# toandaominh1997/EfficientDet.Pytorch

Measured on AMD Instinct MI355X. Metric: images/sec EfficientDet-D0 512px fwd+bwd, higher is better.
Workload: dtype f32_hf16x3_bwd_bf16x3

## Files before the change

efficientdet/pytorch_amd/_lib.py:

```python
import ctypes as C
import os

import torch

HERE = os.path.dirname(os.path.abspath(__file__))
LIB_PATH = os.environ.get('EFFDET_HIP_LIB') or os.path.join(os.path.dirname(os.path.abspath(__file__)), 'libeffdet_hip.so')
MAX_SEG = 5
MAX_CONV_SEG = 10
ABI_VERSION = 11
F32, BF16, F32_BF16X3, F32_SPLIT = 0, 1, 2, 3
F32_HSPLIT = 4
ACT_NONE, ACT_RELU, ACT_SWISH, ACT_SIGMOID = 0, 1, 2, 3
RES_NONE, RES_ADD, RES_RELU_MASK, RES_SWISH_GRAD = 0, 1, 2, 3
TUNE_IGEMM_BIG, TUNE_IGEMM_BIG_MIN_M, TUNE_SPLIT_PERS, TUNE_IGEMM_KORD, TUNE_SPLIT_KORD = 0, 1, 2, 3, 4

_ERR = {-1: 'EFFDET_EINVAL', -2: 'EFFDET_ELAUNCH', -3: 'EFFDET_EUNSUPPORTED'}


class Seg(C.Structure):
    _fields_ = [('H', C.c_int), ('W', C.c_int), ('Ho', C.c_int), ('Wo', C.c_int),
                ('in_off', C.c_longlong), ('in_bstride', C.c_longlong),
                ('out_off', C.c_longlong), ('out_bstride', C.c_longlong)]


class ConvDesc(C.Structure):
    _fields_ = [('x', C.c_void_p), ('w', C.c_void_p), ('y', C.c_void_p), ('z', C.c_void_p), ('res', C.c_void_p),
                ('scale', C.c_void_p), ('shift', C.c_void_p), ('rowscale', C.c_void_p),
                ('bc_scale', C.c_void_p), ('bc_shift', C.c_void_p),
                ('dtype', C.c_int), ('out_f32', C.c_int),
                ('B', C.c_int), ('Cin', C.c_int), ('Cout', C.c_int), ('KH', C.c_int), ('KW', C.c_int),
                ('stride', C.c_int), ('pad_t', C.c_int), ('pad_l', C.c_int),
                ('ldx', C.c_int), ('ldy', C.c_int), ('act', C.c_int), ('res_mode', C.c_int),
                ('nseg', C.c_int), ('seg', Seg * MAX_CONV_SEG), ('w_image_stride', C.c_longlong), ('y_split', C.c_void_p), ('range_flag', C.c_void_p),
                ('seg_w', C.c_void_p * MAX_CONV_SEG), ('seg_shift', C.c_void_p * MAX_CONV_SEG)]


class WgradDesc(C.Structure):
    _fields_ = [('x', C.c_void_p), ('dz', C.c_void_p), ('dw', C.c_void_p), ('dbias', C.c_void_p),
                ('dtype', C.c_int),
                ('B', C.c_int), ('Cin', C.c_int), ('Cout', C.c_int), ('KH', C.c_int), ('KW', C.c_int),
                ('stride', C.c_int), ('pad_t', C.c_int), ('pad_l', C.c_int),
                ('ldx', C.c_int), ('lddz', C.c_int), ('nseg', C.c_int), ('image_splits', C.c_int), ('seg', Seg * MAX_SEG)]


class PrepJob(C.Structure):
    _fields_ = [('a', C.c_void_p), ('b', C.c_void_p), ('c', C.c_void_p), ('d', C.c_void_p), ('out', C.c_void_p),
                ('kind', C.c_int), ('dtype', C.c_int), ('n0', C.c_int), ('n1', C.c_int), ('n2', C.c_int), ('n3', C.c_int),
                ('n4', C.c_int), ('eps', C.c_float)]


class UnpackJob(C.Structure):
    _fields_ = [(n, C.c_void_p) for n in ('g', 'scale', 'w_oihw', 'dw_oihw', 'wsum', 'dsum_part', 'mean', 'invstd', 'dgamma', 'dbeta',
                                          'dbias_out', 'slab_scale', 'slab_cscale')] + \
               [(n, C.c_int) for n in ('accumulate', 'Cout', 'Cin', 'KH', 'KW', 'Cin_pad', 'nslabs', 'slabs_per_scale')]


class SeParamJob(C.Structure):
    _fields_ = [(n, C.c_void_p) for n in ('du', 'dmid', 'sw', 'pool', 'dw1', 'db1', 'dw2', 'db2')] + \
               [('B', C.c_int), ('C', C.c_int), ('Cse', C.c_int), ('inv_hw', C.c_float)]


class DwUnpackJob(C.Structure):
    _fields_ = [(n, C.c_void_p) for n in ('g_kkc', 'scale', 'w_c1kk', 'dw_c1kk', 'wsum', 'dsum', 'mean', 'invstd', 'dgamma', 'dbeta')] + \
               [('C', C.c_int), ('kk', C.c_int)]


class _TailUnion(C.Union):
# ... 296 lines not shown
```

efficientdet/pytorch_amd/csrc/conv_igemm.hip:

```cpp
#include "common.h"
#include "../../../include/effdet_live_tiles.h"
#include "../../../include/effdet_needed_tiles.h"
#include "../../../include/effdet_conv_plan.h"
#include "../../../include/effdet_gate_operand.h"
#include <stdlib.h>

#ifndef EFFDET_IGEMM_BIG_DEFAULT
#define EFFDET_IGEMM_BIG_DEFAULT 1
#endif

namespace {

struct SegD {
  int H, W, Ho, Wo, M, tile_start;
  long long in_off, in_bs, out_off, out_bs;
  unsigned x_bytes;
  long long w_off;
  long long sh_off;
};

struct ConvK {
  const void* x; const void* w; void* y; void* z; const void* res;
  const float* scale; const float* shift; const float* rowscale;
  const float* bc_scale; const float* bc_shift;
  int Cin, Cout, KW, stride, pad_t, pad_l;
  int ldx, ldy;
  int Kc;
  int cpt;
  int act, res_mode, out_f32, vec_ok;
  int out_split;
  int* range_flag;
  void* ysplit;
  int nseg, mtiles, ntiles;
  unsigned w_bytes;
  int kord;
  long long w_img_bytes;
  const unsigned char* live;
  int live_tile0;
  const unsigned char* needed;
  int needed_tile0;
  const float* a_gate;
  SegD seg[EFFDET_MAX_CONV_SEG];
};

constexpr int BM = 128;
typedef float f32x16 __attribute__((ext_vector_type(16)));

template <typename T> struct Mma;
template <> struct Mma<bf16_t> {
  static __device__ __forceinline__ void run(const uint4& a, const uint4& b, f32x4& c) {
    c = __builtin_amdgcn_mfma_f32_16x16x32_bf16(__builtin_bit_cast(bf16x8, a), __builtin_bit_cast(bf16x8, b), c, 0, 0, 0);
  }
};
struct MmaH {
  static __device__ __forceinline__ void run(const uint4& a, const uint4& b, f32x4& c) {
    c = __builtin_amdgcn_mfma_f32_16x16x32_f16(__builtin_bit_cast(f16x8, a), __builtin_bit_cast(f16x8, b), c, 0, 0, 0);
  }
};
template <> struct Mma<float> {
  static __device__ __forceinline__ void run(const uint4& a, const uint4& b, f32x4& c) {
    c = __builtin_amdgcn_mfma_f32_16x16x4f32(__uint_as_float(a.x), __uint_as_float(b.x), c, 0, 0, 0);
    c = __builtin_amdgcn_mfma_f32_16x16x4f32(__uint_as_float(a.y), __uint_as_float(b.y), c, 0, 0, 0);
    c = __builtin_amdgcn_mfma_f32_16x16x4f32(__uint_as_float(a.z), __uint_as_float(b.z), c, 0, 0, 0);
    c = __builtin_amdgcn_mfma_f32_16x16x4f32(__uint_as_float(a.w), __uint_as_float(b.w), c, 0, 0, 0);
  }
};

template <typename T, int BN, int WAVES_N, int NWAVES, int SPLIT = 0, int NS = 2, int M32 = 0, int GATE = 0>
__global__ __launch_bounds__(NWAVES * 64, (SPLIT == 3 && NWAVES == 4) ? 3 : 1) void conv_igemm_kernel(const ConvK p) {
  static_assert(!SPLIT || sizeof(T) == 4, "bf16x3 splitting applies to fp32 storage");
  static_assert(!M32 || SPLIT == 2, "the 32x32x16 form is built for the split layout");
  static_assert(SPLIT != 3 || NS == 2, "f16x3: two stages");
  static_assert(NS == 2 || !M32, "deep staging is not built for the 32x32 tile loop");
  static_assert(!GATE || (SPLIT == 0 && sizeof(T) == 4), "the operand gate is built for the exact-fp32 form");
  constexpr int CE = Elem<T>::CE;
  constexpr int NTHREADS = NWAVES * 64;
  constexpr int WAVES_M = NWAVES / WAVES_N;
  constexpr int WTM = BM / WAVES_M, WTN = BN / WAVES_N;
  constexpr int MT = WTM / 16, NT = WTN / 16;
  constexpr int XLD = BM * 8;
  constexpr int WLD = BN * 8;
  constexpr int RSTEP = NTHREADS / 8;
  constexpr int XROWS = BM / RSTEP;
  constexpr int WROWS = (BN + RSTEP - 1) / RSTEP;

  extern __shared__ __attribute__((aligned(16))) uint4 smem[];
  uint4* xs = smem;
  uint4* ws = smem + NS * XLD;

  const int tid = threadIdx.x;
  const int lane = tid & 63, wave = tid >> 6;
  const int wm0 = (wave / WAVES_N) * WTM, wn0 = (wave % WAVES_N) * WTN;

  int tile = xcd_remap(blockIdx.x, gridDim.x);
  if constexpr (SPLIT == 2) {
    if (p.live) {
      const int b = blockIdx.x, whole = (p.mtiles >> 3) << 3;
      if (b < whole * p.ntiles) {
        const int i = b >> 3, j = i / p.ntiles;
        tile = (j * 8 + (b & 7)) * p.ntiles + (i - j * p.ntiles);
      } else tile = b;
    }
  }
  if constexpr (SPLIT == 3) {
    if (p.needed) {
      const int b = blockIdx.x, whole = (p.mtiles >> 3) << 3;
      if (b < whole * p.ntiles) {
        const int i = b >> 3, j = i / p.ntiles;
        tile = (j * 8 + (b & 7)) * p.ntiles + (i - j * p.ntiles);
      } else tile = b;
    }
  }
  const int mt = tile / p.ntiles, nt = tile - mt * p.ntiles;
  int si = 0;
#pragma unroll
  for (int s = 1; s < EFFDET_MAX_CONV_SEG; ++s)
    if (s < p.nseg && mt >= p.seg[s].tile_start) si = s;
  const SegD sg = p.seg[si];
  const int m_base = (mt - sg.tile_start) * BM;
  const int n_base = nt * BN;
  const int HoWo = sg.Ho * sg.Wo;

  if constexpr (SPLIT == 2) {
    if (p.live && mt >= p.live_tile0 && p.live[mt - p.live_tile0] == 0) {
      if (p.res_mode == EFFDET_RES_ADD) return;
      const int rows = min(BM, sg.M - m_base), nch = min(BN, p.Cout - n_base);
      if (p.vec_ok) {
        const int q4 = nch >> 2;
        for (int i = tid; i < rows * q4; i += NTHREADS) {
          const int row = i / q4, c = i - row * q4;
          const int m = m_base + row, bi = m / HoWo, pix = m - bi * HoWo;
          *(uint4*)((float*)p.y + sg.out_off + (long long)bi * sg.out_bs + (long long)pix * p.ldy + n_base + 4 * c) = make_uint4(0u, 0u, 0u, 0u);
        }
      } else {
        for (int i = tid; i < rows * nch; i += NTHREADS) {
          const int row = i / nch, c = i - row * nch;
          const int m = m_base + row, bi = m / HoWo, pix = m - bi * HoWo;
          ((float*)p.y)[sg.out_off + (long long)bi * sg.out_bs + (long long)pix * p.ldy + n_base + c] = 0.f;
        }
      }
      return;
    }
  }

  if constexpr (SPLIT == 3) {
    if (p.needed && mt >= p.needed_tile0 && p.needed[mt - p.needed_tile0] == 0) {
      const int rows = min(BM, sg.M - m_base), nch = min(BN, p.Cout - n_base);
      if (p.vec_ok) {
        const int q4 = nch >> 2;
        for (int i = tid; i < rows * q4; i += NTHREADS) {
          const int row = i / q4, c = i - row * q4;
          const int m = m_base + row, bi = m / HoWo, pix = m - bi * HoWo;
          const long long o = sg.out_off + (long long)bi * sg.out_bs + (long long)pix * p.ldy + n_base + 4 * c;
          *(uint4*)((float*)p.y + o) = make_uint4(0u, 0u, 0u, 0u);
          if (p.ysplit) *(uint4*)((float*)p.ysplit + o) = make_uint4(0u, 0u, 0u, 0u);
        }
      } else {
        for (int i = tid; i < rows * nch; i += NTHREADS) {
          const int row = i / nch, c = i - row * nch;
          const int m = m_base + row, bi = m / HoWo, pix = m - bi * HoWo;
          ((float*)p.y)[sg.out_off + (long long)bi * sg.out_bs + (long long)pix * p.ldy + n_base + c] = 0.f;
        }
      }
      return;
    }
  }

  constexpr unsigned ES = sizeof(T);
  const long long w_img = p.w_img_bytes ? (long long)(m_base / HoWo) * p.w_img_bytes : 0ll;
  const u32x4_t rx = make_srd_raw((const T*)p.x + sg.in_off, sg.x_bytes), rw = make_srd_raw((const char*)p.w + w_img + sg.w_off, p.w_bytes);
  const unsigned xs_a = lds_addr(xs), ws_a = lds_addr(ws);
  const int kc = (tid & 7) ^ ((tid >> 4) & 7), r0 = tid >> 3;
  const int wrow0 = __builtin_amdgcn_readfirstlane(wave) * 8;
  unsigned xoff[XROWS]; int hi0[XROWS], wi0[XROWS];
#pragma unroll
  for (int j = 0; j < XROWS; ++j) {
    const int m = m_base + r0 + RSTEP * j;
    if (m < sg.M) {
      const int b = m / HoWo, rem = m - b * HoWo;
      const int ho = rem / sg.Wo, wo = rem - ho * sg.Wo;
      hi0[j] = ho * p.stride - p.pad_t; wi0[j] = wo * p.stride - p.pad_l;
      xoff[j] = (unsigned)((long long)b * sg.in_bs * ES);
    } else { hi0[j] = -100000; wi0[j] = 0; xoff[j] = 0; }
  }
  unsigned woff[WROWS]; bool wok[WROWS];
#pragma unroll
  for (int j = 0; j < WROWS; ++j) {
    const int r = r0 + RSTEP * j, n = n_base + r;
    wok[j] = (r < BN) && (n < p.Cout);
    woff[j] = (unsigned)((long long)(wok[j] ? n : 0) * p.Kc * 16);
  }
  int kq = kc, tap = 0, cc = kc;
  while (cc >= p.cpt) { cc -= p.cpt; ++tap; }
  int kh = tap / p.KW, kw = tap - kh * p.KW;
  int tapi = tap;
  unsigned xcur[XROWS];
  auto retap = [&]() {
#pragma unroll
    for (int j = 0; j < XROWS; ++j) {
      const int hi = hi0[j] + kh, wi = wi0[j] + kw;
      const bool ok = hi >= 0 && hi < sg.H && wi >= 0 && wi < sg.W;
      xcur[j] = ok ? xoff[j] + (unsigned)((hi * sg.W + wi) * p.ldx + cc * CE) * ES : EFFDET_OOB;
    }
  };
  retap();

  auto stage = [&](int buf) {
    const bool kok = kq < p.Kc;
#pragma unroll
    for (int j = 0; j < XROWS; ++j)
      dma16_async(rx, xs_a + (unsigned)(buf * XLD + (wrow0 + RSTEP * j) * 8) * 16u, kok ? xcur[j] : EFFDET_OOB);
#pragma unroll
    for (int j = 0; j < WROWS; ++j) {
      if (wrow0 + RSTEP * j < BN)
        dma16_async(rw, ws_a + (unsigned)(buf * WLD + (wrow0 + RSTEP * j) * 8) * 16u, (kok && wok[j]) ? woff[j] + (unsigned)kq * 16u : EFFDET_OOB);
    }
    if constexpr (SPLIT != 1) {
      if (p.kord == 1) {
        const int taps = p.Kc / p.cpt;
        ++tapi;
        if (++kw == p.KW) { kw = 0; ++kh; }
        if (tapi == taps) { tapi = 0; kh = 0; kw = 0; cc += 8; }
        kq = (cc < p.cpt) ? tapi * p.cpt + cc : p.Kc;
        retap();
        return;
      }
    }
    kq += 8; cc += 8;
    if (cc < p.cpt) {
#pragma unroll
      for (int j = 0; j < XROWS; ++j) xcur[j] = (xcur[j] == EFFDET_OOB) ? EFFDET_OOB : xcur[j] + 128u;
    } else {
      while (cc >= p.cpt) { cc -= p.cpt; ++kw; if (kw == p.KW) { kw = 0; ++kh; } }
      retap();
    }
  };

  f32x4 acc[NT][MT];
#pragma unroll
  for (int a = 0; a < NT; ++a)
#pragma unroll
    for (int b = 0; b < MT; ++b) acc[a][b] = f32x4{0.f, 0.f, 0.f, 0.f};

  const int nk = (p.Kc + 7) >> 3;
  const int l15 = lane & 15, lq = lane >> 4, lsw = l15 >> 1;
  float* const gl = (float*)(smem + NS * (XLD + WLD));
  if constexpr (GATE) {
    const float* grow = p.a_gate + (long long)(m_base / HoWo) * p.Cin;
    for (int i = tid; i < nk * 32; i += NTHREADS) gl[i] = i < p.Cin ? grow[i] : 0.f;
  }
  auto load = [&](int buf, int s, uint4 (&wf)[NT], uint4 (&xf)[MT]) {
    const int ch = ((s * 4 + lq) ^ lsw);
#pragma unroll
    for (int a = 0; a < NT; ++a) wf[a] = ws[buf * WLD + (wn0 + a * 16 + l15) * 8 + ch];
#pragma unroll
    for (int b = 0; b < MT; ++b) xf[b] = xs[buf * XLD + (wm0 + b * 16 + l15) * 8 + ch];
  };
  auto mma = [&](const uint4 (&wf)[NT], const uint4 (&xf)[MT]) {
#pragma unroll
    for (int a = 0; a < NT; ++a)
#pragma unroll
      for (int b = 0; b < MT; ++b) Mma<T>::run(wf[a], xf[b], acc[a][b]);
  };
  constexpr int PPS = XROWS + WROWS;
// ... 29 lines not shown
        for (int a = 0; a < NT32; ++a) wh[a] = ws[buf * WLD + (wn0 + a * 32 + l31) * 8 + ch];
#pragma unroll
        for (int b = 0; b < MT32; ++b) xh[b] = xs[buf * XLD + (wm0 + b * 32 + l31) * 8 + ch];
#pragma unroll
        for (int b = 0; b < MT32; ++b) xl[b] = xs[buf * XLD + (wm0 + b * 32 + l31) * 8 + cl];
#pragma unroll
        for (int a = 0; a < NT32; ++a) wl[a] = ws[buf * WLD + (wn0 + a * 32 + l31) * 8 + cl];
#pragma unroll
        for (int t = 0; t < 3; ++t)
#pragma unroll
          for (int a = 0; a < NT32; ++a)
#pragma unroll
            for (int b = 0; b < MT32; ++b) mm32(t == 2 ? wl[a] : wh[a], t == 1 ? xl[b] : xh[b], acc32[a][b]);
      }
    };
    stage(0);
    if (nk > 1) stage(1);
    dma_wait_all();
    __syncthreads();
    for (int kt = 0; kt < nk; ++kt) {
      const int c = kt & 1;
      kstep(c);
      if (kt + 1 < nk) {
        dma_wait_all();
        __syncthreads();
        if (kt + 2 < nk) stage(c);
      }
    }
  } else if constexpr (SPLIT) {
    struct Frags { uint4 wh[NT], wl[NT], xh[MT], xl[MT]; };
    f32x4 acc2[SPLIT == 3 ? NT : 1][SPLIT == 3 ? MT : 1];
    if constexpr (SPLIT == 3) {
#pragma unroll
      for (int a = 0; a < NT; ++a)
#pragma unroll
        for (int b = 0; b < MT; ++b) acc2[a][b] = f32x4{0.f, 0.f, 0.f, 0.f};
    }
    auto split8 = [](const uint4& c0, const uint4& c1, uint4& hi, uint4& lo) {
      const unsigned v[8] = {c0.x, c0.y, c0.z, c0.w, c1.x, c1.y, c1.z, c1.w};
      unsigned h[4], l[4];
#pragma unroll
      for (int i = 0; i < 4; ++i) {
        const float a = __uint_as_float(v[2 * i]), b = __uint_as_float(v[2 * i + 1]);
        h[i] = pack2bf(a, b);
        l[i] = pack2bf(a - __uint_as_float(h[i] << 16), b - __uint_as_float(h[i] & 0xffff0000u));
      }
      hi = make_uint4(h[0], h[1], h[2], h[3]); lo = make_uint4(l[0], l[1], l[2], l[3]);
    };
    auto loadsp = [&](int buf, Frags& f) {
      if constexpr (SPLIT >= 2) {
#pragma unroll
        for (int a = 0; a < NT; ++a) f.wh[a] = ws[buf * WLD + (wn0 + a * 16 + l15) * 8 + (lq ^ lsw)];
#pragma unroll
        for (int b = 0; b < MT; ++b) f.xh[b] = xs[buf * XLD + (wm0 + b * 16 + l15) * 8 + (lq ^ lsw)];
#pragma unroll
        for (int b = 0; b < MT; ++b) f.xl[b] = xs[buf * XLD + (wm0 + b * 16 + l15) * 8 + ((4 + lq) ^ lsw)];
#pragma unroll
        for (int a = 0; a < NT; ++a) f.wl[a] = ws[buf * WLD + (wn0 + a * 16 + l15) * 8 + ((4 + lq) ^ lsw)];
      } else {
#pragma unroll
        for (int a = 0; a < NT; ++a) {
          const int r = buf * WLD + (wn0 + a * 16 + l15) * 8;
          f.wh[a] = ws[r + (lq ^ lsw)]; f.wl[a] = ws[r + ((4 + lq) ^ lsw)];
        }
#pragma unroll
        for (int b = 0; b < MT; ++b) {
          const int r = buf * XLD + (wm0 + b * 16 + l15) * 8;
          split8(xs[r + ((2 * lq) ^ lsw)], xs[r + ((2 * lq + 1) ^ lsw)], f.xh[b], f.xl[b]);
        }
      }
    };
    auto mmasp = [&](const Frags& f) {
#pragma unroll
      for (int t = 0; t < 3; ++t)
#pragma unroll
        for (int a = 0; a < NT; ++a)
#pragma unroll
          for (int b = 0; b < MT; ++b) {
            if constexpr (SPLIT == 3) MmaH::run(t == 2 ? f.wl[a] : f.wh[a], t == 1 ? f.xl[b] : f.xh[b], t == 1 ? acc2[a][b] : acc[a][b]);
            else if constexpr (SPLIT == 2) Mma<bf16_t>::run(t == 2 ? f.wl[a] : f.wh[a], t == 1 ? f.xl[b] : f.xh[b], acc[a][b]);
            else Mma<bf16_t>::run(t == 0 ? f.wl[a] : f.wh[a], t == 1 ? f.xl[b] : f.xh[b], acc[a][b]);
          }
    };
    Frags f;
    int issued = 0;
    for (; issued < NS && issued < nk; ++issued) stage(issued);
    wait_tile(issued - 1);
    __syncthreads();
    for (int kt = 0; kt < nk; ++kt) {
      const int c = kt % NS;
      loadsp(c, f);
      mmasp(f);
      if (kt + 1 < nk) {
        wait_tile(issued - (kt + 2));
        __syncthreads();
        if (issued < nk) { stage(c); ++issued; }
      }
    }
    if constexpr (SPLIT == 3) {
#pragma unroll
      for (int a = 0; a < NT; ++a)
#pragma unroll
        for (int b = 0; b < MT; ++b) acc[a][b] += acc2[a][b] * (1.0f / 2048.0f);
    }
  } else {
    uint4 wfA[NT], xfA[MT], wfB[NT], xfB[MT];
    f32x4 gA = f32x4{0.f, 0.f, 0.f, 0.f}, gB = gA;
    auto loadg = [&](int kt, int s) -> f32x4 { return *(const f32x4*)(gl + ((kt * 8 + s * 4 + lq) << 2)); };
    auto gatex = [&](uint4 (&xf)[MT], const f32x4& g) {
      __builtin_amdgcn_sched_barrier(0);
#pragma unroll
      for (int b = 0; b < MT; ++b) {
        float v[4] = {__uint_as_float(xf[b].x), __uint_as_float(xf[b].y), __uint_as_float(xf[b].z), __uint_as_float(xf[b].w)};
        if constexpr (GATE == 2) {
#pragma unroll
          for (int e = 0; e < 4; ++e) v[e] = swishf_(v[e]);
        }
#pragma unroll
        for (int e = 0; e < 4; ++e) v[e] *= g[e];
        xf[b] = make_uint4(__float_as_uint(v[0]), __float_as_uint(v[1]), __float_as_uint(v[2]), __float_as_uint(v[3]));
      }
    };
    int issued = 0;
    for (; issued < NS && issued < nk; ++issued) stage(issued);
    wait_tile(issued - 1);
    __syncthreads();
    load(0, 0, wfA, xfA);
    if constexpr (GATE) { gA = loadg(0, 0); gatex(xfA, gA); }
    for (int kt = 0; kt + 1 < nk; ++kt) {
      const int cur = kt % NS, nxt = (kt + 1) % NS;
      load(cur, 1, wfB, xfB);
      if constexpr (GATE) gB = loadg(kt, 1);
      __builtin_amdgcn_sched_barrier(0);
      mma(wfA, xfA);
      if constexpr (GATE) gatex(xfB, gB);
      wait_tile(issued - (kt + 2));
      __syncthreads();
      if (issued < nk) { stage(cur); ++issued; }
      load(nxt, 0, wfA, xfA);
      if constexpr (GATE) gA = loadg(kt + 1, 0);
      __builtin_amdgcn_sched_barrier(0);
      mma(wfB, xfB);
      if constexpr (GATE) gatex(xfA, gA);
    }
    load((nk - 1) % NS, 1, wfB, xfB);
    if constexpr (GATE) gB = loadg(nk - 1, 1);
    mma(wfA, xfA);
    if constexpr (GATE) gatex(xfB, gB);
    mma(wfB, xfB);
  }
// ... 596 lines not shown
          const f32x4 xv = xt[cur][pl * C4 + k];
#pragma unroll
          for (int j = 0; j < 4; ++j) {
            const f32x2v xx = f32x2v{xv[j], xv[j]};
            a01 = __builtin_elementwise_fma(w01[4 * k + j], xx, a01);
            a23 = __builtin_elementwise_fma(w23[4 * k + j], xx, a23);
          }
        }
        f32x4 v = f32x4{a01[0], a01[1], a23[0], a23[1]} * sc + sh;
        if (p.z) *(f32x4*)((float*)p.z + o) = v;
        if (p.act == EFFDET_ACT_RELU) { for (int r = 0; r < 4; ++r) v[r] = relu_(v[r]); }
        else if (p.act == EFFDET_ACT_SWISH) { for (int r = 0; r < 4; ++r) v[r] = swishf_(v[r]); }
        else if (p.act == EFFDET_ACT_SIGMOID) { for (int r = 0; r < 4; ++r) v[r] = sigmoidf_(v[r]); }
        if (p.rowscale || p.bc_scale) {
          const int bi = m / HoWo;
          if (p.rowscale) v *= p.rowscale[bi];
          if (p.bc_scale) { const int bo = bi * p.Cout + n0; v = v * *(const f32x4*)(p.bc_scale + bo) + *(const f32x4*)(p.bc_shift + bo); }
        }
        if (p.res_mode == EFFDET_RES_ADD) { v += q; }
        else if (p.res_mode == EFFDET_RES_RELU_MASK) { for (int r = 0; r < 4; ++r) v[r] = relu_bwd_(q[r], v[r]); }
        else if (p.res_mode == EFFDET_RES_SWISH_GRAD) { for (int r = 0; r < 4; ++r) v[r] *= swish_gradf_(q[r]); }
        *(f32x4*)((float*)p.y + o) = v;
      }
    }
    if (tile + 1 < ntile) sstore(cur ^ 1);
    __syncthreads();
  }
}

static bool pw_eligible(const effdet_conv_t* p) {
  static const int on = getenv("EFFDET_CONV_PW") ? atoi(getenv("EFFDET_CONV_PW")) : 1;
  if (!on || p->dtype != EFFDET_F32 || p->out_f32 || p->nseg != 1 || p->KH != 1 || p->KW != 1 || p->stride != 1 || p->pad_t || p->pad_l) return false;
  if ((p->Cin != 16 && p->Cin != 24) || p->Cout % 4 || p->Cout < 32 || p->Cout > 1024) return false;
  const effdet_seg_t& g = p->seg[0];
  if (g.H != g.Ho || g.W != g.Wo || p->ldx != p->Cin || p->ldy != p->Cout) return false;
  if (g.in_bstride != (long long)g.H * g.W * p->ldx || g.out_bstride != (long long)g.Ho * g.Wo * p->ldy) return false;
  if (g.in_off % 4 || g.out_off % 4) return false;
  return (long long)p->B * g.H * g.W >= 65536;
}

struct ConvPlan {
  int id;
  ConvK k;
  int (*launch)(const ConvPlan&, hipStream_t);
  unsigned grid;
  size_t lds;
  int pw_G, pw_NPS, pw_ppw;
  int form, pers;
  int tile_m, tile_n, stages, threads, m32;
  int ksteps;
  int gate;
};

template <typename T, int BN, int WAVES_N, int NWAVES, int SPLIT, int NS, int M32, int GATE>
int launch_igemm(const ConvPlan& c, hipStream_t st) {
  if (c.lds > 48 * 1024) EFFDET_SET_MAX_LDS((conv_igemm_kernel<T, BN, WAVES_N, NWAVES, SPLIT, NS, M32, GATE>), c.lds);
  hipLaunchKernelGGL((conv_igemm_kernel<T, BN, WAVES_N, NWAVES, SPLIT, NS, M32, GATE>), dim3(c.grid), dim3(NWAVES * 64), c.lds, st, c.k);
  EFFDET_CHECK_LAUNCH();
  return EFFDET_OK;
}
template <typename T, int BN, int WAVES_N, int NWAVES, int SPLIT = 0, int NS = 2, int M32 = 0, int GATE = 0>
int use_igemm(ConvPlan& c, int id) {
  c.k.ntiles = (c.k.Cout + BN - 1) / BN;
  c.grid = (unsigned)(c.k.mtiles * c.k.ntiles);
  c.lds = (size_t)NS * (BM + BN) * 8 * sizeof(uint4);
  if (GATE) c.lds += (size_t)((c.k.Kc + 7) >> 3) * 32 * sizeof(float);
  c.gate = GATE;
  c.launch = launch_igemm<T, BN, WAVES_N, NWAVES, SPLIT, NS, M32, GATE>;
  static_assert(EFFDET_CONV_FORM_PLAIN == 0 && EFFDET_CONV_FORM_BF16X3 == 1 && EFFDET_CONV_FORM_SPLIT == 2 && EFFDET_CONV_FORM_HSPLIT == 3,
                "the kernel's SPLIT parameter is the public form code");
  c.form = SPLIT; c.pers = 0; c.tile_m = BM; c.tile_n = BN; c.stages = NS; c.threads = NWAVES * 64; c.m32 = M32;
  c.ksteps = (c.k.Kc + 7) >> 3;
  return c.id = id;
}

template <int WM, int WN, int NS, int X3>
int launch_pers(const ConvPlan& c, hipStream_t st) {
  EFFDET_SET_MAX_LDS((conv_igemm_pers_kernel<WM, WN, NS, X3>), c.lds);
  static unsigned ncu = 0;
  if (ncu == 0) { int dev = 0; hipDeviceProp_t pr; ncu = (hipGetDevice(&dev) == hipSuccess && hipGetDeviceProperties(&pr, dev) == hipSuccess) ? pr.multiProcessorCount : 256; }
  const unsigned grid = c.grid < ncu ? c.grid : ncu;
  hipLaunchKernelGGL((conv_igemm_pers_kernel<WM, WN, NS, X3>), dim3(grid), dim3(WM * WN * 64), c.lds, st, c.k);
  EFFDET_CHECK_LAUNCH();
  return EFFDET_OK;
}
template <int WM, int WN, int NS, int X3 = 0>
int use_pers(ConvPlan& c, int id) {
  constexpr int TM = 64 * WM, TN = 64 * WN;
  ConvK& k = c.k;
  k.mtiles = 0;
  for (int s = 0; s < k.nseg; ++s) { k.seg[s].tile_start = k.mtiles; k.mtiles += (k.seg[s].M + TM - 1) / TM; }
  k.ntiles = (k.Cout + TN - 1) / TN;
  if (X3) {
    k.ldx *= 2;
    for (int s = 0; s < k.nseg; ++s) { k.seg[s].in_off *= 2; k.seg[s].in_bs *= 2; }
  }
  c.grid = (unsigned)(k.mtiles * k.ntiles);
  c.lds = (size_t)NS * (TM + TN) * 128;
  c.launch = launch_pers<WM, WN, NS, X3>;
  c.form = X3 ? EFFDET_CONV_FORM_SPLIT : EFFDET_CONV_FORM_PLAIN; c.pers = 1; c.tile_m = TM; c.tile_n = TN; c.stages = NS; c.threads = WM * WN * 64; c.m32 = 1;
  c.ksteps = (k.Kc / k.cpt) * (k.cpt >> 3);
  return c.id = id;
}
static int use_big(ConvPlan& c, int id) {
  switch (id) {
    case 10 + 442: return use_pers<4, 4, 2>(c, id);
    case 10 + 242: return use_pers<2, 4, 2>(c, id);
    case 10 + 243: return use_pers<2, 4, 3>(c, id);
    case 10 + 4220: return use_pers<4, 2, 2>(c, id);
    default: return use_pers<4, 2, 3>(c, id);
  }
}

template <int CIN>
int launch_pw(const ConvPlan& c, hipStream_t st) {
  hipLaunchKernelGGL(conv_pw_f32_kernel<CIN>, dim3(c.grid), dim3(256), 0, st, c.k, c.k.seg[0].M, c.pw_G, c.pw_NPS, c.pw_ppw);
  EFFDET_CHECK_LAUNCH();
  return EFFDET_OK;
}
static int use_pw(ConvPlan& c) {
  c.pw_G = c.k.Cout / 4; c.pw_NPS = 256 / c.pw_G; c.pw_ppw = 1024;
  c.grid = (unsigned)((c.k.seg[0].M + c.pw_ppw - 1) / c.pw_ppw);
  c.lds = 0;
  c.launch = c.k.Cin == 16 ? launch_pw<16> : launch_pw<24>;
  c.form = EFFDET_CONV_FORM_SKINNY; c.pers = 0; c.tile_m = 64; c.tile_n = c.k.Cout; c.stages = 2; c.threads = 256; c.m32 = 0;
  c.k.mtiles = (int)c.grid; c.k.ntiles = 1; c.ksteps = 1;
  return c.id = 20;
}

static int g_tuning[EFFDET_TUNE_COUNT] = {-1, 16384, -1, 1, -1};
static int big_variant() {
  if (g_tuning[EFFDET_TUNE_IGEMM_BIG] < 0)
    g_tuning[EFFDET_TUNE_IGEMM_BIG] = getenv("EFFDET_IGEMM_BIG") ? atoi(getenv("EFFDET_IGEMM_BIG")) : EFFDET_IGEMM_BIG_DEFAULT;
  return g_tuning[EFFDET_TUNE_IGEMM_BIG];
}

template <typename T, int SPLIT, int GATE = 0>
int use_tile(ConvPlan& c, int bt) {
  const ConvK& k = c.k;
  const int id = bt + (SPLIT ? 4 : 0), bn = 128 >> bt;
  const long long tiles = (long long)k.mtiles * ((k.Cout + bn - 1) / bn);
  static const int deep_env = getenv("EFFDET_IGEMM_DEEP") ? atoi(getenv("EFFDET_IGEMM_DEEP")) : 2;
  if ((SPLIT ? deep_env >= 2 : deep_env >= 1) && tiles <= 256 && k.Kc >= 6 * 8) {
    static const int narrow = getenv("EFFDET_IGEMM_NARROW") ? atoi(getenv("EFFDET_IGEMM_NARROW")) : 128;
    static const int narrow_k = getenv("EFFDET_IGEMM_NARROW_K") ? atoi(getenv("EFFDET_IGEMM_NARROW_K")) : 16;
    if (narrow && bt <= 1 && tiles <= narrow && k.Kc >= narrow_k * 8) return use_igemm<T, 32, 1, 4, SPLIT, 4, 0, GATE>(c, id);
    if (bt == 0) return use_igemm<T, 128, 2, 8, SPLIT, 4, 0, GATE>(c, id);
    if (bt == 1) return use_igemm<T, 64, 1, 4, SPLIT, 4, 0, GATE>(c, id);
  }
  switch (bt) {
    case 0: return use_igemm<T, 128, 2, 8, SPLIT, 2, 0, GATE>(c, id);
    case 1: return use_igemm<T, 64, 1, 4, SPLIT, 2, 0, GATE>(c, id);
    case 2: return use_igemm<T, 32, 1, 4, SPLIT, 2, 0, GATE>(c, id);
    default: return use_igemm<T, 16, 1, 4, SPLIT, 2, 0, GATE>(c, id);
  }
}

}

extern "C" int effdet_tuning_set(int key, int value) {
  if (key < 0 || key >= EFFDET_TUNE_COUNT) return EFFDET_EINVAL;
  (void)big_variant();
  const int old = g_tuning[key];
  g_tuning[key] = value;
  return old;
}

static int plan_conv(const effdet_conv_t* p, ConvPlan& c, const float* a_gate = nullptr, int a_act = EFFDET_ACT_NONE) {
  ConvK& k = c.k;
  c.gate = 0;
  if (!p || !p->x || !p->w || !p->y) return EFFDET_EINVAL;
  if (p->nseg < 1 || p->nseg > EFFDET_MAX_CONV_SEG) return EFFDET_EINVAL;
  if (p->dtype != EFFDET_F32 && p->dtype != EFFDET_BF16 && p->dtype != EFFDET_F32_BF16X3 && p->dtype != EFFDET_F32_SPLIT && p->dtype != EFFDET_F32_HSPLIT) return EFFDET_EINVAL;
  const int ce = p->dtype == EFFDET_BF16 ? 8 : 4;
  if (p->Cin % ce || p->ldx % ce || p->KH < 1 || p->KW < 1 || p->stride < 1) return EFFDET_EUNSUPPORTED;
  if (p->res_mode != EFFDET_RES_NONE && !p->res) return EFFDET_EINVAL;
  const bool hfmt = p->dtype == EFFDET_F32_HSPLIT;
  const bool splitfmt = p->dtype == EFFDET_F32_SPLIT || hfmt;
  if (hfmt && (p->res_mode != EFFDET_RES_NONE || p->scale || p->bc_scale || p->rowscale || p->w_image_stride || (p->KH * p->KW * p->Cin) % 32)) return EFFDET_EUNSUPPORTED;
  if (splitfmt) {
    if (p->Cin % 32 || p->ldx % 32 || p->z) return EFFDET_EUNSUPPORTED;
    if (p->out_f32 ? (p->res_mode != EFFDET_RES_NONE && p->res_mode != EFFDET_RES_ADD)
                   : (p->Cout % 32 || p->ldy % 32 || (p->res_mode != EFFDET_RES_NONE && p->res_mode != EFFDET_RES_RELU_MASK))) return EFFDET_EUNSUPPORTED;
    for (int s = 0; s < p->nseg; ++s) {
      if (p->seg[s].in_off % 32 || p->seg[s].in_bstride % 32) return EFFDET_EUNSUPPORTED;
      if (!p->out_f32 && (p->seg[s].out_off % 32 || p->seg[s].out_bstride % 32)) return EFFDET_EUNSUPPORTED;
    }
  } else if (p->out_f32 && (p->z || p->res_mode != EFFDET_RES_NONE)) return EFFDET_EUNSUPPORTED;
  if (p->y_split) {
    if ((p->dtype != EFFDET_F32 && !hfmt) || p->out_f32 || p->res_mode != EFFDET_RES_NONE || p->Cout % 32 || p->ldy % 32) return EFFDET_EUNSUPPORTED;
    for (int s = 0; s < p->nseg; ++s)
      if (p->seg[s].out_off % 32 || p->seg[s].out_bstride % 32) return EFFDET_EUNSUPPORTED;
  }
  k.x = p->x; k.w = p->w; k.y = p->y; k.z = p->z; k.res = p->res; k.ysplit = p->y_split; k.range_flag = hfmt ? p->range_flag : nullptr;
  k.scale = p->scale; k.shift = p->shift; k.rowscale = p->rowscale;
  k.bc_scale = p->bc_scale; k.bc_shift = p->bc_shift;
  if ((p->bc_scale != nullptr) != (p->bc_shift != nullptr)) return EFFDET_EINVAL;
  k.Cin = p->Cin; k.Cout = p->Cout; k.KW = p->KW; k.stride = p->stride; k.pad_t = p->pad_t; k.pad_l = p->pad_l;
  k.ldx = p->ldx; k.ldy = p->ldy;
  k.cpt = p->Cin / ce; k.Kc = p->KH * p->KW * k.cpt;
  k.act = p->act; k.res_mode = p->res_mode; k.out_f32 = p->out_f32; k.kord = g_tuning[EFFDET_TUNE_IGEMM_KORD];
  k.out_split = (splitfmt && !p->out_f32) ? 1 : 0;
  if (splitfmt) {
    if (g_tuning[EFFDET_TUNE_SPLIT_KORD] < 0) g_tuning[EFFDET_TUNE_SPLIT_KORD] = getenv("EFFDET_SPLIT_KORD") ? atoi(getenv("EFFDET_SPLIT_KORD")) : 1;
    const int kv = g_tuning[EFFDET_TUNE_SPLIT_KORD];
    k.kord = ((kv == 1 || (kv == 2 && p->Cout <= 64)) && k.cpt % 8 == 0) ? 1 : 0;
  }
  k.nseg = p->nseg;
  k.w_img_bytes = p->w_image_stride;
  k.live = nullptr; k.live_tile0 = 0;
  k.needed = nullptr; k.needed_tile0 = 0;
  k.a_gate = a_gate;
  if (a_gate) {
    if (a_act != EFFDET_ACT_NONE && a_act != EFFDET_ACT_SWISH) return EFFDET_EINVAL;
    if (p->dtype != EFFDET_F32 || p->KH != 1 || p->KW != 1 || p->stride != 1 || p->pad_t || p->pad_l || p->nseg != 1 || p->w_image_stride ||
        p->seg[0].H != p->seg[0].Ho || p->seg[0].W != p->seg[0].Wo || (p->seg[0].Ho * p->seg[0].Wo) % BM || ((size_t)a_gate & 3)) return EFFDET_EUNSUPPORTED;
  }
  if (p->w_image_stride) {
    if (p->w_image_stride < 0 || (p->w_image_stride & 15) || p->nseg != 1 || splitfmt || (p->seg[0].Ho * p->seg[0].Wo) % BM) return EFFDET_EUNSUPPORTED;
  }
  int tiles = 0;
  bool per_seg = false;
  bool vec = (p->ldy % 4 == 0) && (p->Cout % 4 == 0);
  for (int s = 0; s < p->nseg; ++s) {
    const effdet_seg_t& g = p->seg[s];
    SegD& d = k.seg[s];
    d.H = g.H; d.W = g.W; d.Ho = g.Ho; d.Wo = g.Wo;
    d.M = p->B * g.Ho * g.Wo;
    d.tile_start = tiles;
    d.in_off = g.in_off; d.in_bs = g.in_bstride; d.out_off = g.out_off; d.out_bs = g.out_bstride;
    d.w_off = p->seg_w[s] ? (long long)((const char*)p->seg_w[s] - (const char*)p->w) : 0ll;
    d.sh_off = p->seg_shift[s] ? (long long)(p->seg_shift[s] - p->shift) : 0ll;
    if (p->seg_w[s] || p->seg_shift[s]) per_seg = true;
    if ((p->seg_shift[s] && !p->shift) || (d.w_off & 15)) return EFFDET_EINVAL;
    if (d.M <= 0) return EFFDET_EINVAL;
    if (g.in_off % ce || g.in_bstride % ce) return EFFDET_EUNSUPPORTED;
    if (g.out_off % 4 || g.out_bstride % 4) vec = false;
    tiles += (d.M + BM - 1) / BM;
  }
  for (int s = p->nseg; s < EFFDET_MAX_CONV_SEG; ++s) { k.seg[s] = k.seg[0]; k.seg[s].tile_start = 0x7fffffff; }
  k.mtiles = tiles; k.vec_ok = vec ? 1 : 0;
  if (per_seg && (p->w_image_stride || p->scale)) return EFFDET_EUNSUPPORTED;
  const long long es = p->dtype == EFFDET_BF16 ? 2 : 4;
  for (int s = 0; s < p->nseg; ++s) {
    const effdet_seg_t& g = p->seg[s];
    const long long e = ((long long)(p->B - 1) * g.in_bstride + ((long long)(g.H - 1) * g.W + (g.W - 1)) * p->ldx + p->Cin) * es;
    if (e >= 0xFFFF0000LL) return EFFDET_EUNSUPPORTED;
    k.seg[s].x_bytes = (unsigned)e;
  }
  const long long wb = (long long)p->Cout * k.Kc * 16;
  if (wb >= 0xFFFF0000LL) return EFFDET_EUNSUPPORTED;
  k.w_bytes = (unsigned)wb;
  if (hfmt) {
    k.scale = (const float*)((const char*)p->w + wb);
    return p->Cout > 64 ? use_igemm<float, 128, 2, 8, 3>(c, 30) : use_igemm<float, 64, 1, 4, 3>(c, 31);
  }
  long long mtot = 0;
  bool fits = true;
  for (int s = 0; s < p->nseg; ++s) {
    mtot += k.seg[s].M;
    if ((long long)k.seg[s].x_bytes + 2LL * ((long long)p->KH * p->seg[s].W + p->KW) * p->ldx * es >= 0x70000000LL) fits = false;
  }
  if (p->dtype == EFFDET_BF16 && !per_seg && !p->bc_scale && !p->w_image_stride && p->Cin % 64 == 0 && p->KH * p->KW <= 32 && p->Cout >= 128 && big_variant() != 0 && wb < 0x40000000LL &&
      fits && mtot >= g_tuning[EFFDET_TUNE_IGEMM_BIG_MIN_M]) {
    const int v = big_variant();
// ... 97 lines not shown
```

include/effdet_hip.h:

```cpp
#ifndef EFFDET_HIP_H
#define EFFDET_HIP_H
#ifdef __cplusplus
extern "C" {
#endif

typedef void* effdet_stream_t;

enum { EFFDET_OK = 0, EFFDET_EINVAL = -1, EFFDET_ELAUNCH = -2, EFFDET_EUNSUPPORTED = -3 };
enum { EFFDET_F32 = 0, EFFDET_BF16 = 1,
       EFFDET_F32_BF16X3 = 2,
       EFFDET_F32_SPLIT = 3,
       EFFDET_F32_HSPLIT = 4 };
enum { EFFDET_ACT_NONE = 0, EFFDET_ACT_RELU = 1, EFFDET_ACT_SWISH = 2, EFFDET_ACT_SIGMOID = 3 };
enum { EFFDET_RES_NONE = 0, EFFDET_RES_ADD = 1, EFFDET_RES_RELU_MASK = 2, EFFDET_RES_SWISH_GRAD = 3 };

#define EFFDET_MAX_SEG 5
#define EFFDET_MAX_CONV_SEG 10

typedef struct {
  int H, W, Ho, Wo;
  long long in_off, in_bstride, out_off, out_bstride;
} effdet_seg_t;

typedef struct {
  const void* x; const void* w; void* y; void* z; const void* res;
  const float* scale; const float* shift;
  const float* rowscale;
  const float* bc_scale; const float* bc_shift;
  int dtype, out_f32;
  int B, Cin, Cout, KH, KW, stride, pad_t, pad_l;
  int ldx, ldy;
  int act, res_mode;
  int nseg;
  effdet_seg_t seg[EFFDET_MAX_CONV_SEG];
  long long w_image_stride;
  void* y_split;
  int* range_flag;
  const void* seg_w[EFFDET_MAX_CONV_SEG];
  const float* seg_shift[EFFDET_MAX_CONV_SEG];
} effdet_conv_t;
int effdet_conv2d(const effdet_conv_t* p, effdet_stream_t stream);
int effdet_scale_pack_weight(const float* w, const float* gate, void* out, int dtype, int B, int Cout, int Cin, effdet_stream_t stream);

int effdet_conv2d_kernel(const effdet_conv_t* p);

enum { EFFDET_TUNE_IGEMM_BIG = 0, EFFDET_TUNE_IGEMM_BIG_MIN_M = 1,
       EFFDET_TUNE_SPLIT_PERS = 2 ,
       EFFDET_TUNE_IGEMM_KORD = 3 ,
       EFFDET_TUNE_SPLIT_KORD = 4 , EFFDET_TUNE_COUNT = 5 };
int effdet_tuning_set(int key, int value);

typedef struct {
  const void* x; const void* dz; float* dw; float* dbias;
  int dtype;
  int B, Cin, Cout, KH, KW, stride, pad_t, pad_l;
  int ldx, lddz;
  int nseg;
  int image_splits;
  effdet_seg_t seg[EFFDET_MAX_SEG];
} effdet_wgrad_t;
long long effdet_conv2d_wgrad_workspace_bytes(const effdet_wgrad_t* p);
int effdet_conv2d_wgrad_splits(const effdet_wgrad_t* p);
int effdet_conv2d_wgrad_seg_slabs(const effdet_wgrad_t* p, int* first, int* count);
int effdet_conv2d_wgrad_kernel(const effdet_wgrad_t* p);
int effdet_conv2d_wgrad(const effdet_wgrad_t* p, void* workspace, long long workspace_bytes, effdet_stream_t stream);

int effdet_pack_conv_weight(const float* w_oihw, const float* scale, void* out, int dtype, int mode,
                            int Cout, int Cin, int KH, int KW, int Cin_pad, effdet_stream_t stream);
int effdet_unpack_conv_wgrad(const float* g, const float* scale, const float* w_oihw, float* dw_oihw,
                             float* wsum, int accumulate, int Cout, int Cin, int KH, int KW, int Cin_pad, int nslabs,
                             const float* dbias_part, float* dbias_out, const float* slab_scale, int slabs_per_scale,
                             effdet_stream_t stream);
int effdet_unpack_conv_wgrad_bn(const float* g, const float* scale, const float* w_oihw, float* dw_oihw, const float* dsum_part,
                                const float* mean, const float* invstd, float* dgamma, float* dbeta, int Cout, int Cin,
                                int KH, int KW, int Cin_pad, int nslabs, const float* slab_scale, int slabs_per_scale,
                                effdet_stream_t stream);

typedef struct {
  const float* g; const float* scale; const float* w_oihw; float* dw_oihw; float* wsum;
  const float* dsum_part; const float* mean; const float* invstd; float* dgamma; float* dbeta; float* dbias_out;
  const float* slab_scale;
  const float* slab_cscale;
  int accumulate, Cout, Cin, KH, KW, Cin_pad, nslabs, slabs_per_scale;
} effdet_unpack_job_t;
int effdet_unpack_conv_wgrad_batch(const effdet_unpack_job_t* jobs, int njobs, effdet_stream_t stream);

enum { EFFDET_TAIL_UNPACK = 0, EFFDET_TAIL_SE_PARAMS = 1, EFFDET_TAIL_DW_UNPACK = 2 };
typedef struct {
  const float* du; const float* dmid; const float* sw; const float* pool;
  float* dw1; float* db1; float* dw2; float* db2;
  int B, C, Cse; float inv_hw;
} effdet_se_param_job_t;
typedef struct {
  const float* g_kkc; const float* scale; const float* w_c1kk; float* dw_c1kk; float* wsum;
  const float* dsum; const float* mean; const float* invstd; float* dgamma; float* dbeta;
  int C, kk;
} effdet_dw_unpack_job_t;
typedef struct {
  int kind;
  union { effdet_unpack_job_t conv; effdet_se_param_job_t se; effdet_dw_unpack_job_t dw; } u;
} effdet_tail_job_t;
int effdet_backward_tail(const effdet_tail_job_t* jobs, int njobs, effdet_stream_t stream);
// ... 257 lines not shown
```

Baseline: 1388.

## Stage padded row slabs once per channel group for 3x3 split-precision convs

For stride-1 3x3 convs in the split-precision implicit-GEMM path (kord==1), the kernel now loads a padded slab of whole image rows (BM/W rows plus halo columns) into LDS once per kh and channel group. It reuses that slab across the three kw taps by shifting LDS indices, instead of gathering a fresh im2col tile for every tap. Weights get their own staging walk and custom waitcnt accounting. This cuts global x traffic and DMA issue roughly threefold for those layers, at the cost of a larger LDS footprint, more complex synchronisation and a new env/tuning switch that defaults to on.

```diff
diff --git a/efficientdet/pytorch_amd/_lib.py b/efficientdet/pytorch_amd/_lib.py
--- a/efficientdet/pytorch_amd/_lib.py
+++ b/efficientdet/pytorch_amd/_lib.py
@@ -13,6 +13,7 @@
 ACT_NONE, ACT_RELU, ACT_SWISH, ACT_SIGMOID = 0, 1, 2, 3
 RES_NONE, RES_ADD, RES_RELU_MASK, RES_SWISH_GRAD = 0, 1, 2, 3
 TUNE_IGEMM_BIG, TUNE_IGEMM_BIG_MIN_M, TUNE_SPLIT_PERS, TUNE_IGEMM_KORD, TUNE_SPLIT_KORD = 0, 1, 2, 3, 4
+TUNE_ROWSLAB = 5
 
 _ERR = {-1: 'EFFDET_EINVAL', -2: 'EFFDET_ELAUNCH', -3: 'EFFDET_EUNSUPPORTED'}
 
diff --git a/efficientdet/pytorch_amd/csrc/conv_igemm.hip b/efficientdet/pytorch_amd/csrc/conv_igemm.hip
--- a/efficientdet/pytorch_amd/csrc/conv_igemm.hip
+++ b/efficientdet/pytorch_amd/csrc/conv_igemm.hip
@@ -40,10 +40,17 @@
   const unsigned char* needed;
   int needed_tile0;
   const float* a_gate;
+  int slab;
+  int xld;
   SegD seg[EFFDET_MAX_CONV_SEG];
 };
 
 constexpr int BM = 128;
+
+__host__ __device__ inline int slab_entries(int W) { return (BM / W) * (W + 2); }
+__host__ __device__ inline bool slab_seg_ok(const SegD& s, int bn) {
+  return (s.W & (s.W - 1)) == 0 && s.W >= (bn > 64 ? 8 : 16) && s.W <= 64 && s.Ho == s.H && s.Wo == s.W;
+}
 typedef float f32x16 __attribute__((ext_vector_type(16)));
 
 template <typename T> struct Mma;
@@ -84,9 +91,15 @@
   constexpr int XROWS = BM / RSTEP;
   constexpr int WROWS = (BN + RSTEP - 1) / RSTEP;
 
+  constexpr bool SLABCAP = SPLIT >= 2 && NS == 2 && !M32;
+  constexpr int SP = SLABCAP ? (160 + RSTEP - 1) / RSTEP : 1;
+  static_assert(!SLABCAP || ((SP - 1) * RSTEP == 128 && WROWS * RSTEP == BN), "slab passes: 128 entries for every wave, the rest in the last pass");
+  static_assert(!SLABCAP || MT <= 2, "slab fragments: fragment 1 is one uniform entry step from fragment 0");
+
   extern __shared__ __attribute__((aligned(16))) uint4 smem[];
-  uint4* xs = smem;
-  uint4* ws = smem + NS * XLD;
+  const int xld = SLABCAP ? p.xld : XLD;
+  uint4* xs = SLABCAP ? smem + NS * WLD : smem;
+  uint4* ws = SLABCAP ? smem : smem + NS * XLD;
 
   const int tid = threadIdx.x;
   const int lane = tid & 63, wave = tid >> 6;
@@ -172,11 +185,12 @@
   const unsigned xs_a = lds_addr(xs), ws_a = lds_addr(ws);
   const int kc = (tid & 7) ^ ((tid >> 4) & 7), r0 = tid >> 3;
   const int wrow0 = __builtin_amdgcn_readfirstlane(wave) * 8;
+  const bool slab = SLABCAP && p.slab && slab_seg_ok(sg, BN);
   unsigned xoff[XROWS]; int hi0[XROWS], wi0[XROWS];
 #pragma unroll
   for (int j = 0; j < XROWS; ++j) {
     const int m = m_base + r0 + RSTEP * j;
-    if (m < sg.M) {
+    if (m < sg.M && !slab) {
       const int b = m / HoWo, rem = m - b * HoWo;
       const int ho = rem / sg.Wo, wo = rem - ho * sg.Wo;
       hi0[j] = ho * p.stride - p.pad_t; wi0[j] = wo * p.stride - p.pad_l;
@@ -209,7 +223,7 @@
     const bool kok = kq < p.Kc;
 #pragma unroll
     for (int j = 0; j < XROWS; ++j)
-      dma16_async(rx, xs_a + (unsigned)(buf * XLD + (wrow0 + RSTEP * j) * 8) * 16u, kok ? xcur[j] : EFFDET_OOB);
+      dma16_async(rx, xs_a + (unsigned)(buf * xld + (wrow0 + RSTEP * j) * 8) * 16u, kok ? xcur[j] : EFFDET_OOB);
 #pragma unroll
     for (int j = 0; j < WROWS; ++j) {
       if (wrow0 + RSTEP * j < BN)
@@ -345,9 +359,9 @@
 #pragma unroll
         for (int a = 0; a < NT; ++a) f.wh[a] = ws[buf * WLD + (wn0 + a * 16 + l15) * 8 + (lq ^ lsw)];
 #pragma unroll
-        for (int b = 0; b < MT; ++b) f.xh[b] = xs[buf * XLD + (wm0 + b * 16 + l15) * 8 + (lq ^ lsw)];
-#pragma unroll
-        for (int b = 0; b < MT; ++b) f.xl[b] = xs[buf * XLD + (wm0 + b * 16 + l15) * 8 + ((4 + lq) ^ lsw)];
+        for (int b = 0; b < MT; ++b) f.xh[b] = xs[buf * xld + (wm0 + b * 16 + l15) * 8 + (lq ^ lsw)];
+#pragma unroll
+        for (int b = 0; b < MT; ++b) f.xl[b] = xs[buf * xld + (wm0 + b * 16 + l15) * 8 + ((4 + lq) ^ lsw)];
 #pragma unroll
         for (int a = 0; a < NT; ++a) f.wl[a] = ws[buf * WLD + (wn0 + a * 16 + l15) * 8 + ((4 + lq) ^ lsw)];
       } else {
@@ -376,6 +390,96 @@
           }
     };
     Frags f;
+    bool walked = false;
+    if constexpr (SLABCAP) {
+      if (slab) {
+        const int W = sg.W, W2 = W + 2, lw = 31 - __builtin_clz((unsigned)W), R = BM >> lw;
+        const int npieces = (R * W2 + 7) >> 3;
+        const bool slast = (wrow0 >> 3) + (SP - 1) * NWAVES < npieces;
+        const int grow0 = m_base >> lw, nrows = sg.M >> lw;
+        const int rowb = W * p.ldx * (int)ES;
+        unsigned sbase[SP], vmask = 0u;
+#pragma unroll
+        for (int j = 0; j < SP; ++j) {
+          const int e = r0 + RSTEP * j, rt = e / W2, w = e - rt * W2 - 1, g = grow0 + rt;
+          const bool ok = rt < R && w >= 0 && w < W && g < nrows;
+          const int b = g / sg.H, h = g - b * sg.H;
+          sbase[j] = (unsigned)((long long)b * sg.in_bs * ES) + (unsigned)((h * W + w) * p.ldx) * ES + (unsigned)kc * 16u;
+          if (ok) vmask |= ((h > 0 ? 1u : 0u) | 2u | (h + 1 < sg.H ? 4u : 0u)) << (3 * j);
+        }
+        const int pt0 = wm0 + l15, ebase = (pt0 >> lw) * W2 + (pt0 & (W - 1)), estep = (16 >> lw) * W2 + (16 & (W - 1));
+        int s_kh = 0, s_g = 0;
+        auto stage_slab = [&](int buf) {
+          const unsigned walk = (unsigned)((s_kh - 1) * rowb + s_g * 128);
+#pragma unroll
+          for (int j = 0; j < SP; ++j) {
+            if (j < SP - 1 || slast)
+              dma16_async(rx, xs_a + (unsigned)(buf * xld + (wrow0 + RSTEP * j) * 8) * 16u, ((vmask >> (3 * j + s_kh)) & 1u) ? sbase[j] + walk : EFFDET_OOB);
+          }
+          if (++s_kh == 3) { s_kh = 0; ++s_g; }
+        };
+#pragma unroll
+        for (int j = 0; j < WROWS; ++j) woff[j] += (unsigned)kc * 16u;
+        int w_g = 0;
+        auto stage_w = [&](int buf) {
+          const bool kok = w_g * 8 < p.cpt;
+          const unsigned walk = (unsigned)(tapi * p.cpt + w_g * 8) * 16u;
+#pragma unroll
+          for (int j = 0; j < WROWS; ++j)
+            dma16_async(rw, ws_a + (unsigned)(buf * WLD + (wrow0 + RSTEP * j) * 8) * 16u, (kok && wok[j]) ? woff[j] + walk : EFFDET_OOB);
+          if (++tapi == 9) { tapi = 0; ++w_g; }
+        };
+        auto wait_keep = [&](bool w1) {
+          if (w1) {
+            if (slast) asm volatile("s_waitcnt vmcnt(%0)" :: "n"(SP + WROWS) : "memory");
+            else asm volatile("s_waitcnt vmcnt(%0)" :: "n"(SP - 1 + WROWS) : "memory");
+          } else {
+            if (slast) asm volatile("s_waitcnt vmcnt(%0)" :: "n"(SP) : "memory");
+            else asm volatile("s_waitcnt vmcnt(%0)" :: "n"(SP - 1) : "memory");
+          }
+        };
+        auto loadslab = [&](int wbuf, int sbuf, int kw3, Frags& fr) {
+          int xi[MT];
+#pragma unroll
+          for (int b = 0; b < MT; ++b) {
+            const int e = ebase + b * estep + kw3;
+            xi[b] = sbuf * xld + e * 8 + (lq ^ ((e >> 1) & 7));
+          }
+#pragma unroll
+          for (int a = 0; a < NT; ++a) fr.wh[a] = ws[wbuf * WLD + (wn0 + a * 16 + l15) * 8 + (lq ^ lsw)];
+#pragma unroll
+          for (int b = 0; b < MT; ++b) fr.xh[b] = xs[xi[b]];
+#pragma unroll
+          for (int b = 0; b < MT; ++b) fr.xl[b] = xs[xi[b] ^ 4];
+#pragma unroll
+          for (int a = 0; a < NT; ++a) fr.wl[a] = ws[wbuf * WLD + (wn0 + a * 16 + l15) * 8 + ((4 + lq) ^ lsw)];
+        };
+        const int nslab = nk / 3;
+        int issued = 2, sissued = 1, kw3 = 0, sbuf = 0;
+        bool inflight = false;
+        stage_slab(0); stage_w(0); stage_w(1);
+        if (nslab > 1) { stage_slab(1); sissued = 2; inflight = true; wait_keep(true); }
+        else dma_wait_all();
+        __syncthreads();
+        for (int kt = 0; kt < nk; ++kt) {
+          const int c = kt & 1;
+          loadslab(c, sbuf, kw3, f);
+          mmasp(f);
+          if (kt + 1 < nk) {
+            if (kw3 == 0 && inflight) wait_keep(false);
+            else { dma_wait_all(); inflight = false; }
+            __syncthreads();
+            if (issued < nk) { stage_w(c); ++issued; }
+            if (kw3 == 2) {
+              if (sissued < nslab) { stage_slab(sbuf); ++sissued; inflight = true; }
+              sbuf ^= 1; kw3 = 0;
+            } else ++kw3;
+          }
+        }
+        walked = true;
+      }
+    }
+    if (!walked) {
     int issued = 0;
     for (; issued < NS && issued < nk; ++issued) stage(issued);
     wait_tile(issued - 1);
@@ -389,6 +493,7 @@
         __syncthreads();
         if (issued < nk) { stage(c); ++issued; }
       }
+    }
     }
     if constexpr (SPLIT == 3) {
 #pragma unroll
@@ -1091,6 +1196,12 @@
   int gate;
 };
 
+static int g_tuning[EFFDET_TUNE_COUNT] = {-1, 16384, -1, 1, -1, -1};
+static bool rowslab_on() {
+  if (g_tuning[EFFDET_TUNE_ROWSLAB] < 0) g_tuning[EFFDET_TUNE_ROWSLAB] = getenv("EFFDET_ROWSLAB") ? atoi(getenv("EFFDET_ROWSLAB")) : 1;
+  return g_tuning[EFFDET_TUNE_ROWSLAB] != 0;
+}
+
 template <typename T, int BN, int WAVES_N, int NWAVES, int SPLIT, int NS, int M32, int GATE>
 int launch_igemm(const ConvPlan& c, hipStream_t st) {
   if (c.lds > 48 * 1024) EFFDET_SET_MAX_LDS((conv_igemm_kernel<T, BN, WAVES_N, NWAVES, SPLIT, NS, M32, GATE>), c.lds);
@@ -1102,7 +1213,17 @@
 int use_igemm(ConvPlan& c, int id) {
   c.k.ntiles = (c.k.Cout + BN - 1) / BN;
   c.grid = (unsigned)(c.k.mtiles * c.k.ntiles);
-  c.lds = (size_t)NS * (BM + BN) * 8 * sizeof(uint4);
+  c.k.slab = 0; c.k.xld = BM * 8;
+  if constexpr (SPLIT >= 2 && NS == 2 && !M32) {
+    const ConvK& k = c.k;
+    if (rowslab_on() && k.kord == 1 && k.KW == 3 && k.Kc == 9 * k.cpt && k.stride == 1 && k.pad_t == 1 && k.pad_l == 1) {
+      int ent = 0;
+      for (int s = 0; s < k.nseg; ++s)
+        if (slab_seg_ok(k.seg[s], BN) && ((slab_entries(k.seg[s].W) + 7) & ~7) > ent) ent = (slab_entries(k.seg[s].W) + 7) & ~7;
+      if (ent) { c.k.slab = 1; c.k.xld = (ent > BM ? ent : BM) * 8; }
+    }
+  }
+  c.lds = (size_t)NS * (c.k.xld + BN * 8) * sizeof(uint4);
   if (GATE) c.lds += (size_t)((c.k.Kc + 7) >> 3) * 32 * sizeof(float);
   c.gate = GATE;
   c.launch = launch_igemm<T, BN, WAVES_N, NWAVES, SPLIT, NS, M32, GATE>;
@@ -1167,7 +1288,6 @@
   return c.id = 20;
 }
 
-static int g_tuning[EFFDET_TUNE_COUNT] = {-1, 16384, -1, 1, -1};
 static int big_variant() {
   if (g_tuning[EFFDET_TUNE_IGEMM_BIG] < 0)
     g_tuning[EFFDET_TUNE_IGEMM_BIG] = getenv("EFFDET_IGEMM_BIG") ? atoi(getenv("EFFDET_IGEMM_BIG")) : EFFDET_IGEMM_BIG_DEFAULT;
@@ -1250,6 +1370,7 @@
   k.live = nullptr; k.live_tile0 = 0;
   k.needed = nullptr; k.needed_tile0 = 0;
   k.a_gate = a_gate;
+  k.slab = 0; k.xld = BM * 8;
   if (a_gate) {
     if (a_act != EFFDET_ACT_NONE && a_act != EFFDET_ACT_SWISH) return EFFDET_EINVAL;
     if (p->dtype != EFFDET_F32 || p->KH != 1 || p->KW != 1 || p->stride != 1 || p->pad_t || p->pad_l || p->nseg != 1 || p->w_image_stride ||
diff --git a/include/effdet_hip.h b/include/effdet_hip.h
--- a/include/effdet_hip.h
+++ b/include/effdet_hip.h
@@ -47,7 +47,9 @@
 enum { EFFDET_TUNE_IGEMM_BIG = 0, EFFDET_TUNE_IGEMM_BIG_MIN_M = 1,
        EFFDET_TUNE_SPLIT_PERS = 2 ,
        EFFDET_TUNE_IGEMM_KORD = 3 ,
-       EFFDET_TUNE_SPLIT_KORD = 4 , EFFDET_TUNE_COUNT = 5 };
+       EFFDET_TUNE_SPLIT_KORD = 4 ,
+       EFFDET_TUNE_ROWSLAB = 5 ,
+       EFFDET_TUNE_COUNT = 6 };
 int effdet_tuning_set(int key, int value);
 
 typedef struct {
```

Result: faster. 1426 (median of 6 runs) (+2.7%).
